# thu-nics/Rad-NeRF

Hardware: AMD Instinct MI355X
Metric: million samples/s fwd+bwd, 8192 rays, model_zoo_size=2; rgb L∞ vs ref (higher is better)
Workload: dtype f16/f32

## Files before the change

### include/radnerf.h

```cpp
#ifndef RADNERF_H
#define RADNERF_H

#include <stdint.h>

#ifdef __cplusplus
extern "C" {
#endif

#define RN_ABI_VERSION 9
#define RN_FX_STATS_BYTES 640
int rn_version(void);
const char* rn_last_error(void);
const char* rn_abi_signatures(void);
void rn_set_debug_flags(int flags);
int rn_debug_cycles(unsigned long long* out);
int rn_set_level_pairing(uint64_t pairing);

int rn_ray_aabb_intersect(const float* rays_o, const float* rays_d, const float* centers,
                          const float* half_sizes, int64_t n_rays, int64_t n_voxels,
                          int32_t max_hits, int32_t* hit_cnt, float* hits_t,
                          int64_t* hits_voxel_idx, void* stream);

int rn_ray_sphere_intersect(const float* rays_o, const float* rays_d, const float* centers,
                            const float* radii, int64_t n_rays, int64_t n_spheres,
// ... 73 lines not shown
                       const float* ts, const int32_t* counts, const int32_t* offsets,
                       int64_t n_rays, int32_t n_models, float T_threshold, int32_t* used,
                       float* opacity_k, float* depth_k, float* rgb_k, float* ws, void* stream);
int rn_ml_combine_fw(const float* gate, const float* opacity_k, const float* depth_k,
                     const float* rgb_k, const float* bg, int64_t n_rays, int32_t n_models,
                     float* rgb, float* opacity, float* depth, void* stream);
int rn_ml_combine_bw(const float* dL_drgb, const float* dL_dopacity, const float* opacity_k,
                     const float* rgb_k, const float* bg, int64_t n_rays, int32_t n_models,
                     float* dL_dgate, void* stream);
int rn_ml_composite_bw(const float* dL_drgb, const float* dL_dopacity, const float* dL_ddepth,
                       const float* gate, const float* bg, const float* sigmas,
                       const float* rgbs, const float* deltas, const float* ts,
                       const int32_t* counts, const int32_t* offsets, const float* opacity_k,
                       const float* depth_k, const float* rgb_k, int64_t n_rays,
                       int32_t n_models, float T_threshold, float* dL_dsigmas, float* dL_drgbs,
                       void* stream);
int rn_ml_composite_dist_fw(const float* sigmas, const float* rgbs, const float* deltas,
                            const float* ts, const int32_t* counts, const int32_t* offsets,
                            int64_t n_rays, int32_t n_models, float T_threshold, int32_t* used,
                            float* opacity_k, float* depth_k, float* rgb_k, float* ws,
                            float* dist_k, void* stream);
int rn_ml_composite_dist_bw(const float* dL_drgb, const float* dL_dopacity,
                            const float* dL_ddepth, const float* dL_ddist, float dL_ddist_const,
                            const float* gate, const float* bg, const float* sigmas,
                            const float* rgbs, const float* deltas, const float* ts,
                            const float* ws, const int32_t* counts, const int32_t* offsets,
                            const float* opacity_k, const float* depth_k, const float* rgb_k,
                            const float* dist_k, int64_t n_rays, int32_t n_models,
                            float T_threshold, float* dL_dsigmas, float* dL_drgbs, void* stream);

int rn_field_fwd(const float* xyzs, const float* dirs, int64_t n_samples, const float* ts,
                 const int32_t* ray_of, const float* rays_o, const float* rays_d,
                 const int32_t* seg_base, const int32_t* seg_count, int32_t n_models,
                 const void* grid_f16, const uint32_t* level_offset, const uint32_t* level_hsize,
                 const uint32_t* level_res, const float* level_scale, const float* xyz_min,
                 const float* extent, const void* frags, float* sigma, float* rgb,
                 void* feat_cache, int32_t blocks_per_model, void* stream);
int rn_field_bwd(const float* xyzs, const float* dirs, int64_t n_samples, const float* ts,
                 const int32_t* ray_of, const float* rays_o, const float* rays_d,
                 const int32_t* seg_base, const int32_t* seg_count, int32_t n_models,
                 const void* grid_f16, const uint32_t* level_offset, const uint32_t* level_hsize,
                 const uint32_t* level_res, const float* level_scale, const float* xyz_min,
                 const float* extent, const void* frags, const float* dL_dsigma,
                 const float* dL_drgb, float* grid_grad, float* dw, const void* feat_cache,
                 int32_t blocks_per_model, void* stream);

int rn_bwd_plan(const int32_t* counts, const int32_t* offsets, const int32_t* seg_base,
                const int32_t* seg_count, const float* ts, int64_t n_rays, int32_t n_models,
                int32_t head_chunks, int32_t head_size, int32_t max_chunk, int32_t min_chunk,
                int32_t balance_blocks, int32_t cap_chunks, int32_t* mstart, int32_t* perm,
                int32_t* chunk_first, int32_t* chunk_desc, int32_t* queue, const float* rays_o,
                const float* rays_d, const float* xyz_min, const float* extent, float* prep,
                void* stream);
int rn_field_bwd_merged(const float* ts, const int32_t* ray_of, const float* rays_o,
                        const float* rays_d, const int32_t* seg_base, const int32_t* seg_count,
                        const int32_t* mstart, const int32_t* perm,
                        const int32_t* chunk_desc, int32_t* queue, int64_t n_rays,
                        int32_t n_models, int32_t max_samples,
                        const void* grid_f16, const uint32_t* level_offset,
                        const uint32_t* level_hsize, const uint32_t* level_res,
                        const float* level_scale, const float* xyz_min, const float* extent,
                        const void* frags, const float* dL_dsigma, const float* dL_drgb,
                        float* grid_grad, float* dw, const void* feat_cache, float* scratch,
                        int64_t scratch_rows, float* park, int32_t max_chunk, int32_t blocks,
                        int32_t* igrad_lo, int32_t* igrad_carry, const float* igrad_scale,
                        int32_t* fx_acc, const float* fx_scale, uint32_t* fx_stats,
                        const int32_t* fx_redo, int32_t fx_mode, void* gb_ctl,
                        uint32_t* gb_page_meta, uint64_t* gb_pages, int32_t gb_pool_pages,
                        void* stream);

int rn_grid_fx_fold(const uint32_t* level_offset, const uint32_t* level_hsize,
                    const uint32_t* level_res, int32_t* fx_acc, const float* fx_scale_cur,
                    float* fx_scale_next, uint32_t* fx_vmax, int32_t* fx_redo, float* grid_grad,
                    void* stream);

int rn_debug_gb_cycles(unsigned long long* out);
int rn_grid_bin_layout(int32_t* out);
int rn_grid_slice_bits(const uint32_t* level_hsize, int32_t* out);
int rn_grid_record_encode(const float* x, int64_t n, uint32_t* out);
int rn_grid_record_decode(const uint32_t* f, int64_t n, int64_t* out);
int rn_grid_bin(const uint32_t* level_hsize, void* ctl, const uint32_t* page_meta,
                const uint64_t* pages_in, uint64_t* pages_out, uint32_t* desc,
                uint32_t* level_pages, int32_t pool_pages, int32_t blocks, void* stream);
int rn_grid_bin_check(const uint32_t* level_hsize, void* ctl, const uint32_t* page_meta,
                      const uint64_t* pages_in, uint64_t* pages_out, uint32_t* desc,
                      uint32_t* level_pages, int32_t pool_pages, const float* fx_scale_cur,
                      float* fx_scale_next, uint32_t* fx_stats, int32_t* fx_redo, void* stream);
int rn_grid_binned_fold(const uint32_t* level_offset, const uint32_t* level_hsize, void* ctl,
                        const uint32_t* page_meta, const uint64_t* pages_in, uint64_t* pages_out,
                        uint32_t* desc, uint32_t* level_pages, int32_t pool_pages,
                        const float* fx_scale_cur, float* fx_scale_next, uint32_t* fx_stats,
                        int32_t* fx_redo, float* grid_grad, void* stream);
int rn_grid_sum(const uint32_t* level_offset, const uint32_t* level_hsize, const void* ctl,
                const uint32_t* desc, const uint32_t* level_pages, const uint64_t* pages_out,
                int32_t pool_pages, const float* fx_scale, const int32_t* redo, float* grid_grad,
                int32_t level_lo, int32_t level_hi, void* stream);

int rn_render_test(const float* rays_o, const float* rays_d, const float* hits_t, int64_t n_rays,
                   int32_t n_models, const uint8_t* density_bitfields, int64_t bitfield_bytes,
                   int32_t cascades, float scale, float exp_step_factor, int32_t grid_size,
                   int32_t max_samples, const void* grid_f16, const uint32_t* level_offset,
                   const uint32_t* level_hsize, const uint32_t* level_res,
                   const float* level_scale, const float* xyz_min, const float* extent,
                   const void* frags, float T_threshold, float* opacity, float* depth,
                   float* rgb, int32_t* n_samples, int32_t blocks, void* stream);

// ... 247 lines not shown
```

### rad-nerf_amd/csrc/field_plan.hip

```cpp
#include "rn_field.h"
#include "rn_merge.h"
#pragma clang fp contract(off)

namespace {

#define PLAN_WAVES 4
#define PLAN_LDS 2048

#define PLAN_UNR 8

struct PlanPrep {
    float4* prep;
    const float* rays_o; const float* rays_d;
    float mn[3], ext[3];
    float inv[3];
};
struct RayPos { float o[3], d[3]; };
__device__ __forceinline__ RayPos plan_ray(const PlanPrep& P, int r) {
    RayPos q;
#pragma unroll
    for (int c = 0; c < 3; ++c) { q.o[c] = P.rays_o[3 * r + c]; q.d[c] = P.rays_d[3 * r + c]; }
    return q;
}
__device__ __forceinline__ void plan_prep_write(const PlanPrep& P, const RayPos& q, int pos,
                                                float t, int s) {
    const float x = fmaf(t, q.d[0], q.o[0]), y = fmaf(t, q.d[1], q.o[1]), z = fmaf(t, q.d[2], q.o[2]);
    auto u = [&](float v, int c) {
        return P.inv[0] != 0.f ? fminf(fmaxf((v - P.mn[c]) * P.inv[c], 0.0f), 1.0f)
                               : unit_coord(v, P.mn[c], P.ext[c]);
    };
    P.prep[pos] = make_float4(u(x, 0), u(y, 1), u(z, 2), __int_as_float(s));
}

__device__ __forceinline__ void plan_ray_runs(int K, int B, int r, const int32_t* __restrict__ counts,
                                              const int32_t* __restrict__ offsets,
                                              const int32_t* __restrict__ seg_base, int* cnt,
                                              int* off, int& ms) {
    int c[MB_KMAX], o[MB_KMAX], sb[MB_KMAX];
#pragma unroll
    for (int k = 0; k < MB_KMAX; ++k) {
        const int kk = k < K ? k : K - 1;
        c[k] = counts[kk * B + r]; o[k] = offsets[kk * B + r]; sb[k] = seg_base[kk];
    }
    ms = 0;
#pragma unroll
    for (int k = 0; k < MB_KMAX; ++k) {
        cnt[k] = k < K ? c[k] : 0;
        off[k] = k < K ? o[k] : 0;
        ms += k < K ? o[k] - sb[k] : 0;
    }
}
__device__ __forceinline__ void plan_stage(int K, int tot_r, const int* bnd, const int* off,
                                           const float* __restrict__ ts, float* st, uint16_t* si) {
    const int lane = rn_lane();
    for (int i0 = 0; i0 < tot_r; i0 += RN_WAVE * PLAN_UNR) {
        float v[PLAN_UNR];
#pragma unroll
        for (int u = 0; u < PLAN_UNR; ++u) {
            const int i = i0 + u * RN_WAVE + lane;
            int base = off[0];
#pragma unroll
            for (int kq = 1; kq < MB_KMAX; ++kq)
                base = (kq < K && i >= bnd[kq]) ? off[kq] - bnd[kq] : base;
            v[u] = i < tot_r ? ts[base + i] : 0.f;
        }
#pragma unroll
        for (int u = 0; u < PLAN_UNR; ++u) {
            const int i = i0 + u * RN_WAVE + lane;
            if (i < tot_r) {
                st[i] = v[u];
                if (si) si[i] = (uint16_t)i;
            }
        }
    }
}

__global__ void __launch_bounds__(PLAN_WAVES * 64)
k_bwd_plan(int B, int K, const int32_t* __restrict__ counts, const int32_t* __restrict__ offsets,
           const int32_t* __restrict__ seg_base, const int32_t* __restrict__ seg_count,
           const float* __restrict__ ts, int32_t* __restrict__ mstart, int32_t* __restrict__ perm,
           PlanPrep P) {
    __shared__ float sT[PLAN_WAVES][PLAN_LDS];
    const int wid = __builtin_amdgcn_readfirstlane(threadIdx.x / RN_WAVE);
    const int r = blockIdx.x * PLAN_WAVES + wid;
    if (r >= B) return;
    const int lane = rn_lane();
    int ms = 0, tot_r = 0;
    int cnt[MB_KMAX], off[MB_KMAX], loc[MB_KMAX];
    plan_ray_runs(K, B, r, counts, offsets, seg_base, cnt, off, ms);
#pragma unroll
    for (int k = 0; k < MB_KMAX; ++k) { loc[k] = tot_r; tot_r += cnt[k]; }
    if (lane == 0) {
        mstart[r] = ms;
        if (r == 0) {
            int tot = 0;
            for (int k = 0; k < K; ++k) tot += seg_count[k];
            mstart[B] = tot;
        }
    }
    const bool staged = tot_r <= PLAN_LDS;
    float* st = sT[wid];
    const RayPos rq = P.prep ? plan_ray(P, r) : RayPos{};
    if (staged) {
        plan_stage(K, tot_r, loc, off, ts, st, nullptr);
        __builtin_amdgcn_wave_barrier();
        __builtin_amdgcn_fence(__ATOMIC_ACQ_REL, "wavefront");
    }
    if (K == 2 && staged) {
        const float* A = st + loc[0];
        const float* Bv = st + loc[1];
        const int nA = cnt[0], nB = cnt[1], n = nA + nB;
        const int L = (n + RN_WAVE - 1) / RN_WAVE;
        const int d = min(lane * L, n);
        int lo = max(0, d - nB), hi = min(d, nA);
        while (lo < hi) {
            const int mid = (lo + hi) >> 1;
            if (A[mid] <= Bv[d - 1 - mid]) lo = mid + 1; else hi = mid;
        }
        int a = lo, b = d - lo;
        const int e = min(d + L, n);
        for (int q = d; q < e; ++q) {
            const bool takeA = a < nA && (b >= nB || A[a] <= Bv[b]);
            const int smp = takeA ? off[0] + a : off[1] + b;
            perm[ms + q] = smp;
            if (P.prep) plan_prep_write(P, rq, ms + q, takeA ? A[a] : Bv[b], smp);
            a += takeA ? 1 : 0;
            b += takeA ? 0 : 1;
        }
        return;
    }
    for (int k = 0; k < K; ++k) {
        for (int i = lane; i < cnt[k]; i += RN_WAVE) {
            const float t = staged ? st[loc[k] + i] : ts[off[k] + i];
            int pos = i;
            for (int k2 = 0; k2 < K; ++k2) {
                if (k2 == k) continue;
                int lo = 0, hi = cnt[k2];
                while (lo < hi) {
                    const int mid = (lo + hi) >> 1;
                    const float t2 = staged ? st[loc[k2] + mid] : ts[off[k2] + mid];
                    if (t2 < t || (k2 < k && t2 == t)) lo = mid + 1; else hi = mid;
                }
                pos += lo;
            }
            perm[ms + pos] = off[k] + i;
            if (P.prep) plan_prep_write(P, rq, ms + pos, t, off[k] + i);
        }
    }
}

#define PLANM_WAVES 2
#define PLANM_LDS 2048

__device__ __forceinline__ void merge_pair_wave(const float* tA, const uint16_t* iA, int nA,
                                                const float* tB, const uint16_t* iB, int nB,
                                                float* to, uint16_t* io, int32_t* gout,
                                                const int* kb, const int* ko, int K,
                                                const PlanPrep& P, const RayPos& rq, int gpos) {
    const int lane = rn_lane();
    const int n = nA + nB;
    const int L = (n + RN_WAVE - 1) / RN_WAVE;
    const int d = min(lane * L, n);
    int lo = max(0, d - nB), hi = min(d, nA);
    while (lo < hi) {
        const int mid = (lo + hi) >> 1;
        if (tA[mid] <= tB[d - 1 - mid]) lo = mid + 1; else hi = mid;
    }
    int a = lo, b = d - lo;
    const int e = min(d + L, n);
    for (int q = d; q < e; ++q) {
        const float ta = tA[a], tb = tB[b];
        const int ja = iA[a], jb = iB[b];
        const bool takeA = a < nA && (b >= nB || ta <= tb);
        const int idx = takeA ? ja : jb;
        if (gout) {
            int base = ko[0];
#pragma unroll
            for (int j = 1; j < MB_KMAX; ++j)
                if (j < K && idx >= kb[j]) base = ko[j] - kb[j];
            gout[q] = base + idx;
            if (P.prep) plan_prep_write(P, rq, gpos + q, takeA ? ta : tb, base + idx);
        } else {
            to[q] = takeA ? ta : tb;
            io[q] = (uint16_t)idx;
        }
        a += takeA ? 1 : 0;
        b += takeA ? 0 : 1;
    }
}

__global__ void __launch_bounds__(PLANM_WAVES * 64)
k_bwd_plan_multi(int B, int K, const int32_t* __restrict__ counts,
                 const int32_t* __restrict__ offsets, const int32_t* __restrict__ seg_base,
                 const int32_t* __restrict__ seg_count, const float* __restrict__ ts,
                 int32_t* __restrict__ mstart, int32_t* __restrict__ perm, PlanPrep P) {
    __shared__ float sT[PLANM_WAVES][2][PLANM_LDS + 2];
    __shared__ uint16_t sI[PLANM_WAVES][2][PLANM_LDS + 2];
    static_assert(PLANM_LDS <= 65536, "u16 sample ids");
    const int wid = __builtin_amdgcn_readfirstlane(threadIdx.x / RN_WAVE);
    const int r = blockIdx.x * PLANM_WAVES + wid;
    if (r >= B) return;
    const int lane = rn_lane();
    int ms = 0, tot_r = 0;
    int bnd[MB_KMAX + 1], off[MB_KMAX], cnt[MB_KMAX];
    plan_ray_runs(K, B, r, counts, offsets, seg_base, cnt, off, ms);
#pragma unroll
    for (int k = 0; k < MB_KMAX; ++k) { bnd[k] = tot_r; tot_r += cnt[k]; }
    bnd[MB_KMAX] = tot_r;
    const RayPos rq = P.prep ? plan_ray(P, r) : RayPos{};
    if (lane == 0) {
        mstart[r] = ms;
        if (r == 0) {
            int tot = 0;
            for (int k = 0; k < K; ++k) tot += seg_count[k];
            mstart[B] = tot;
        }
    }
    if (tot_r > PLANM_LDS) {
        for (int k = 0; k < K; ++k) {
            const int ck = bnd[k + 1] - bnd[k];
            for (int i = lane; i < ck; i += RN_WAVE) {
                const float t = ts[off[k] + i];
                int pos = i;
                for (int k2 = 0; k2 < K; ++k2) {
                    if (k2 == k) continue;
                    int lo = 0, hi = bnd[k2 + 1] - bnd[k2];
                    while (lo < hi) {
                        const int mid = (lo + hi) >> 1;
                        const float t2 = ts[off[k2] + mid];
                        if (t2 < t || (k2 < k && t2 == t)) lo = mid + 1; else hi = mid;
                    }
                    pos += lo;
                }
                perm[ms + pos] = off[k] + i;
                if (P.prep) plan_prep_write(P, rq, ms + pos, t, off[k] + i);
            }
        }
        return;
    }
    int cur = 0;
    int kb[MB_KMAX];
#pragma unroll
    for (int k = 0; k < MB_KMAX; ++k) kb[k] = k < K ? bnd[k] : 0;
    plan_stage(K, tot_r, bnd, off, ts, sT[wid][0], sI[wid][0]);
    int nr = K;
    while (true) {
        __builtin_amdgcn_wave_barrier();
        __builtin_amdgcn_fence(__ATOMIC_ACQ_REL, "wavefront");
        const bool last = nr <= 2;
        const float* ts_ = sT[wid][cur];
        const uint16_t* is_ = sI[wid][cur];
        for (int p = 0; 2 * p < nr; ++p) {
            const int a0 = bnd[2 * p], a1 = bnd[min(2 * p + 1, nr)], b1 = bnd[min(2 * p + 2, nr)];
            merge_pair_wave(ts_ + a0, is_ + a0, a1 - a0, ts_ + a1, is_ + a1, b1 - a1,
                            sT[wid][cur ^ 1] + a0, sI[wid][cur ^ 1] + a0,
                            nullptr, kb, off, K, P, rq, ms + a0);
        }
        if (last) {
            __builtin_amdgcn_wave_barrier();
            __builtin_amdgcn_fence(__ATOMIC_ACQ_REL, "wavefront");
            const float* to = sT[wid][cur ^ 1];
            const uint16_t* io = sI[wid][cur ^ 1];
            for (int q = lane; q < tot_r; q += RN_WAVE) {
                const int idx = io[q];
                int base = off[0];
#pragma unroll
                for (int jk = 1; jk < MB_KMAX; ++jk)
                    if (jk < K && idx >= kb[jk]) base = off[jk] - kb[jk];
                perm[ms + q] = base + idx;
                if (P.prep) plan_prep_write(P, rq, ms + q, to[q], base + idx);
            }
            return;
        }
        const int nn = (nr + 1) / 2;
        for (int p = 0; p < nn; ++p) bnd[p] = bnd[2 * p];
        bnd[nn] = bnd[nr];
        nr = nn;
        cur ^= 1;
    }
}

struct ChunkPlan {
    int head_n, head, max_chunk, min_chunk, c1, n;
    __host__ __device__ int hbound(int c) const {
        return head_n > 0 ? (int)(((int64_t)head * c * (c + 1)) / (2 * (int64_t)head_n)) : 0;
    }
    __host__ __device__ int bound(int c) const {
        const int H = hbound(head_n);
        if (c < head_n) return hbound(c);
        if (c <= c1) return H + (c - head_n) * max_chunk;
        return H + (c1 - head_n) * max_chunk + (c - c1) * min_chunk;
    }
};

__host__ __device__ __forceinline__ ChunkPlan chunk_plan(int total, int head_n, int head,
                                                         int max_chunk, int min_chunk, int blocks) {
    ChunkPlan p;
// ... 8 lines not shown
    if (blocks > 0 && main_end > H) {
        const int64_t main = main_end - H, per = (int64_t)blocks * max_chunk;
        const int64_t m = (main + per - 1) / per;
        const int64_t sz = (main + (int64_t)blocks * m - 1) / ((int64_t)blocks * m);
        p.max_chunk = (int)(sz < min_chunk ? min_chunk : (sz > max_chunk ? max_chunk : sz));
    }
    p.c1 = p.head_n + (main_end > H ? (main_end - H) / p.max_chunk : 0);
    const int rest = total - p.bound(p.c1);
    p.n = p.c1 + (rest > 0 ? (rest + min_chunk - 1) / min_chunk : 0);
    return p;
}

__global__ void __launch_bounds__(256)
k_bwd_chunks(int B, int K, const int32_t* __restrict__ mstart,
             const int32_t* __restrict__ offsets, const int32_t* __restrict__ seg_base,
             const int32_t* __restrict__ seg_count, int head_n, int head, int max_chunk,
             int min_chunk, int blocks, int cap_chunks, int32_t* __restrict__ chunk_first,
             int32_t* __restrict__ desc, int32_t* __restrict__ queue) {
    const int c = blockIdx.x * blockDim.x + threadIdx.x;
    const int total = mstart[B];
    const ChunkPlan p = chunk_plan(total, head_n, head, max_chunk, min_chunk, blocks);
    const int n = min(p.n, cap_chunks);
    if (c == 0) { queue[0] = 0; queue[1] = n; queue[2] = 0; }
    if (c > n) return;
    auto first_ray = [&](int cc) {
        if (cc == p.n) return B;
        const int bound = p.bound(cc);
        int lo = 0, hi = B;
        while (lo < hi) {
            const int mid = (lo + hi) >> 1;
            if (mstart[mid] < bound) lo = mid + 1; else hi = mid;
        }
        return lo;
    };
    if (c == n) { chunk_first[c] = first_ray(c); return; }
    const int first[2] = {first_ray(c), first_ray(c + 1)};
    chunk_first[c] = first[0];
    int32_t* d = desc + (size_t)c * CH_DESC;
    const int r0 = first[0], r1 = first[1];
    d[CH_R0] = r0; d[CH_R1] = r1; d[2] = 0; d[3] = 0;
    for (int k = 0; k < MB_KMAX; ++k) {
        int a0 = 0, cnt = 0;
        if (k < K && r0 < B) {
            a0 = offsets[k * B + r0];
            const int a1 = r1 < B ? offsets[k * B + r1] : seg_base[k] + seg_count[k];
            cnt = a1 - a0;
        }
        d[ch_first(k)] = a0; d[ch_count(k)] = cnt;
    }
}

}

extern "C" {

int rn_bwd_plan(const int32_t* counts, const int32_t* offsets, const int32_t* seg_base,
                const int32_t* seg_count, const float* ts, int64_t n_rays, int32_t n_models,
                int32_t head_chunks, int32_t head_size, int32_t max_chunk, int32_t min_chunk,
                int32_t balance_blocks, int32_t cap_chunks, int32_t* mstart, int32_t* perm,
                int32_t* chunk_first, int32_t* chunk_desc, int32_t* queue, const float* rays_o,
                const float* rays_d, const float* xyz_min, const float* extent, float* prep,
                void* stream) {
    RN_CHECK_ARG(n_rays >= 1 && n_models >= 1 && n_models <= MB_KMAX, "bad sizes");
    RN_CHECK_ARG(max_chunk >= min_chunk && min_chunk >= 1 && cap_chunks >= 1 && head_chunks >= 0 &&
                 head_size >= 0 && head_size <= max_chunk && balance_blocks >= 0,
                 "bad chunk sizes");
    RN_CHECK_ARG(counts && offsets && seg_base && seg_count && ts && mstart && perm &&
                 chunk_first && chunk_desc && queue, "null pointer");
    RN_CHECK_ARG(!prep || (rays_o && rays_d && xyz_min && extent), "null pointer (prep)");
    PlanPrep P{};
    P.prep = (float4*)prep; P.rays_o = rays_o; P.rays_d = rays_d;
    if (prep) {
        bool pow2 = true;
        for (int c = 0; c < 3; ++c) {
            P.mn[c] = xyz_min[c]; P.ext[c] = extent[c];
            int e;
            pow2 = pow2 && extent[c] > 0.f && std::frexp(extent[c], &e) == 0.5f &&
                   e > -120 && e < 120;
        }
        for (int c = 0; c < 3; ++c) P.inv[c] = pow2 ? 1.0f / extent[c] : 0.f;
    }
    if (n_models > 2)
        k_bwd_plan_multi<<<nblk(n_rays, PLANM_WAVES), PLANM_WAVES * 64, 0, (hipStream_t)stream>>>(
            (int)n_rays, n_models, counts, offsets, seg_base, seg_count, ts, mstart, perm, P);
    else
        k_bwd_plan<<<nblk(n_rays, PLAN_WAVES), PLAN_WAVES * 64, 0, (hipStream_t)stream>>>(
            (int)n_rays, n_models, counts, offsets, seg_base, seg_count, ts, mstart, perm, P);
    RN_CHECK_LAUNCH();
    k_bwd_chunks<<<nblk(cap_chunks + 1, 256), 256, 0, (hipStream_t)stream>>>(
        (int)n_rays, n_models, mstart, offsets, seg_base, seg_count, head_chunks, head_size,
        max_chunk, min_chunk, balance_blocks, cap_chunks, chunk_first, chunk_desc, queue);
    RN_CHECK_LAUNCH();
    return 0;
}

}
```

### rad-nerf_amd/radnerf_amd/_lib.py

```python
import ctypes
import os

_HERE = os.path.dirname(os.path.abspath(__file__))
LIB_PATH = os.environ.get("RADNERF_LIB", os.path.join(_HERE, "librn.so"))
ABLATION_LIB_PATH = os.environ.get("RADNERF_ABL_LIB", os.path.join(_HERE, "librn_abl.so"))

P = ctypes.c_void_p
I32 = ctypes.c_int32
I64 = ctypes.c_int64
F32 = ctypes.c_float
F64 = ctypes.c_double
U64 = ctypes.c_uint64

SIGNATURES = {
    "rn_ray_aabb_intersect": [P, P, P, P, I64, I64, I32, P, P, P, P],
    "rn_ray_sphere_intersect": [P, P, P, P, I64, I64, I32, P, P, P, P],
    "rn_raymarching_train_bw": [P, P, P, P, I64, P, P, P],
    "rn_ml_march_bw": [P, P, I64, I32, P, P, P, P, P, P],
    "rn_field_dinput": [P, P, I64, P, P, P, P, P, P, I32, P, P, P, P, P, P, P, P, P, P, P, P, P,
                        P, I32, P],
    "rn_field_density": [P, I64, P, P, P, P, P, P, P, P, P, P, P],
    "rn_debug_cycles": [P],
    "rn_set_level_pairing": [ctypes.c_uint64],
    "rn_density_update_sampled": [P, P, I32, I32, I32, F32, F32, F32, U64, P, P, P, P, P, P, P,
                                  P, P, P, P, P, P, I32, P],
    "rn_density_update_visible": [P, P, I32, I32, I32, F32, F32, F32, U64, P, P, P, P, P, P, P,
                                  P, P, P, P, P, P, I32, P, I32, P],
    "rn_distortion_loss_fw": [P, P, P, P, I64, P, P, P, P],
    "rn_distortion_loss_bw": [P, P, P, P, P, P, P, I64, P, P],
    "rn_raymarching_train_count": [P, P, P, P, I32, F32, F32, P, I32, I32, I64, P, P],
    "rn_raymarching_train_write": [P, P, P, P, I32, F32, F32, P, I32, I32, I64, P, P, P, P, P,
                                   P, P, P],
    "rn_scan_segments": [P, I32, I64, I32, P, P, P, P, P],
    "rn_raymarching_test": [P, P, P, P, I64, P, I32, F32, F32, I32, I32, I32, P, P, P, P, P, P],
    "rn_ml_march_count": [P, P, P, P, F32, P, P, I64, I32, I32, F32, F32, I32, I32, I64, P, P, P,
                          P],
    "rn_ml_compact": [P, P, I64, I32, I32, P, P, P, P, P, P],
    "rn_ml_march_write": [P, P, P, P, F32, P, P, I64, I32, I32, F32, F32, I32, I32, I64, P, P,
                          P, P, P, P],
    "rn_composite_train_fw": [P, P, P, P, P, I64, F32, P, P, P, P, P, P],
    "rn_composite_train_bw": [P, P, P, P, P, P, P, P, P, P, I64, P, P, P, F32, P, P, P],
    "rn_composite_test_fw": [P, P, P, P, I64, I32, P, F32, P, P, P, P, P],
    "rn_ml_composite_fw": [P, P, P, P, P, P, I64, I32, F32, P, P, P, P, P, P],
    "rn_ml_combine_fw": [P, P, P, P, P, I64, I32, P, P, P, P],
    "rn_ml_combine_bw": [P, P, P, P, P, I64, I32, P, P],
    "rn_ml_composite_bw": [P, P, P, P, P, P, P, P, P, P, P, P, P, P, I64, I32, F32, P, P, P],
    "rn_ml_composite_dist_fw": [P, P, P, P, P, P, I64, I32, F32, P, P, P, P, P, P, P],
    "rn_ml_composite_dist_bw": [P, P, P, P, F32, P, P, P, P, P, P, P, P, P, P, P, P, P, I64, I32,
                                F32, P, P, P],
    "rn_field_fwd": [P, P, I64, P, P, P, P, P, P, I32, P, P, P, P, P, P, P, P, P, P, P, I32, P],
    "rn_field_bwd": [P, P, I64, P, P, P, P, P, P, I32, P, P, P, P, P, P, P, P, P, P, P, P, P,
                     I32, P],
    "rn_bwd_plan": [P, P, P, P, P, I64, I32, I32, I32, I32, I32, I32, I32, P, P, P, P, P,
                    P, P, P, P, P, P],
    "rn_field_bwd_merged": [P, P, P, P, P, P, P, P, P, P, I64, I32, I32, P, P, P, P, P, P,
                            P, P, P, P, P, P, P, P, I64, P, I32, I32, P, P, P, P, P, P,
                            P, I32, P, P, P, I32, P],
    "rn_grid_fx_fold": [P, P, P, P, P, P, P, P, P, P],
    "rn_grid_bin_layout": [P],
    "rn_debug_gb_cycles": [P],
    "rn_grid_slice_bits": [P, P],
    "rn_grid_record_encode": [P, I64, P],
    "rn_grid_record_decode": [P, I64, P],
    "rn_grid_bin": [P, P, P, P, P, P, P, I32, I32, P],
    "rn_grid_sum": [P, P, P, P, P, P, I32, P, P, P, I32, I32, P],
    "rn_grid_bin_check": [P, P, P, P, P, P, P, I32, P, P, P, P, P],
    "rn_grid_binned_fold": [P, P, P, P, P, P, P, P, I32, P, P, P, P, P, P],
    "rn_render_test": [P, P, P, I64, I32, P, I64, I32, F32, F32, I32, I32, P, P, P, P, P, P, P,
                       P, F32, P, P, P, P, I32, P],
    "rn_gate_select": [P, I64, I32, F32, I32, I32, P, P, P, P, P, P, P, P, P, P],
    "rn_render_test_list": [P, P, P, I64, I32, P, I64, I32, F32, F32, I32, I32, P, P, P, P, P, P,
                            P, P, F32, P, P, P, P, P, P, I32, P],
    "rn_ml_march_count_list": [P, P, P, P, F32, P, P, I64, I32, I32, F32, F32, I32, I32, I64, P,
                               P, P, P, P, P],
    "rn_gate_select_bw": [P, P, P, I64, I32, I32, P, P],
    "rn_nerf_loss_routed": [P, P, P, P, P, P, P, I64, I32, F32, F32, F32, P, P, P, P, P, P],
    "rn_nerf_loss_routed_det": [P, P, P, P, P, P, P, I64, I32, F32, F32, F32, P, P, P, P, P, P,
                                P],
    "rn_seed_scale": [P, P, I32, P, P, P, P, P, P],
    "rn_igrad_to_f32": [I64, P, P, P, P, P],
    "rn_field_fwd_merged": [P, P, P, P, P, P, P, P, I64, I32, P, P, P, P, P, P, P, P, P, P, P,
                            P, P, I32, I32, P],
    "rn_field_fwd_levels": [P, P, P, P, P, P, I64, I32, P, P, P, P, P, P, P, P, P, P, P, P, P,
                            P, I64, P, I32, I32, I32, P, P],
    "rn_gate_fwd": [P, P, I32, I64, I32, P, P, P, I32, P],
    "rn_gate_bwd": [P, P, I32, I64, I32, P, P, P, I32, P, P, I32, P],
    "rn_nerf_loss": [P, P, P, P, P, P, I64, I32, F32, F32, F32, P, P, P, P, P, P],
    "rn_adam": [P, P, P, P, I64, F64, F64, F64, F64, I32, F32, P, I64, P],
    "rn_reduce_partials": [P, I32, I64, P, P],
    "rn_colsum_ordered": [P, I64, I32, P, P],
    "rn_field_bwd_merged_det": [P, P, P, P, P, P, P, P, P, P, I64, I32, I32, P, P, P, P, P, P,
                                P, P, P, P, P, P, P, P, I64, P, I32, I32, P, P, P, P],
    "rn_gate_bwd_det": [P, P, I32, I64, I32, P, P, P, I32, P, P, I32, P],
    "rn_nerf_loss_det": [P, P, P, P, P, P, I64, I32, F32, F32, F32, P, P, P, P, P, P, P],
    "rn_get_rays": [P, P, P, P, I64, P, P, P, P, P],
    "rn_get_rays_pose": [P, P, P, P, P, P, I64, P, P, P, P, P],
    "rn_get_rays_pose_bw": [P, P, P, P, P, I64, I64, P, P, P, P, P, P, P],
    "rn_sample_batch": [P, I32, I64, I64, P, P, P, P, P, U64, I64, I32, I64, I32, P, P, P, P, P,
                        P, P, P, P],
    "rn_guided_weights": [P, I64, I32, I32, I32, P, P, P, P],
    "rn_sample_batch_guided": [P, I32, I64, I64, P, P, P, P, P, U64, I64, I32, I64, I32, P, P, P,
                               P, P, P, P, P, I32, I32, I32, F32, P, P, P, P, P],
    "rn_guided_epilogue": [P, P, P, P, I64, I32, I64, P, P, P, P, P, P],
    "rn_guided_refresh": [P, P, P, I64, F32, P],
    "rn_ml_combine_test": [P, P, P, P, P, I64, I32, I64, P, P, P, P, P],
    "rn_image_sse": [P, P, I64, P, P, P],
    "rn_ssim": [P, P, I32, I32, I32, P, P, P, P],
# ... 130 lines not shown
```

### rad-nerf_amd/radnerf_amd/fused.py

```python
import collections

import torch

from . import layout as LY
from . import sparse_gate
from ._lib import GATE_SELECT_WORK_BYTES, lib
from .networks import field_ptrs, model_bitfields

MAX_SAMPLES = 1024
NEAR_DISTANCE = 0.01
SEG_ALIGN = 128
FX_STATS_BYTES = 640
GM_F32, GM_FX, GM_FX_REDO, GM_BIN, GM_BIN_F32 = 0, 2, 3, 4, 5
NO_IG, NO_FX, NO_GB = (None, None, None), (None, None, None, None, GM_F32), (None, None, None, 0)


GB_SUM_FAULT = 18
GB_CTL_READ = GB_SUM_FAULT + 1


def clamp_split(split_level):
    return max(0, min(15, int(split_level)))


# ... 284 lines not shown
        return route_params("FusedMLRenderer", self.gate.out_dim, gate_topk, gate_min,
                            renormalize, self._route_always)

    def forward(self, rays_o, rays_d, gate_in2, noise, bg, T_threshold=1e-4,
                exp_step_factor=0.0, distortion=False, gate_topk=None, gate_min=0.0,
                renormalize=False):
        m, g, w, L = self.model, self.gate, self.ws, lib()
        B, K, G = rays_o.shape[0], m.size, g.out_dim
        assert B == w.B and noise.shape == (K, B)
        routed = self._routed = self.route_params(gate_topk, gate_min, renormalize)
        st = _stream(rays_o.device)
        out_gate = torch.empty(B, G, device=rays_o.device)
        imp = torch.zeros(G, device=rays_o.device)
        side = self._side(rays_o.device)
        main = torch.cuda.current_stream(rays_o.device)
        if G == 1:
            out_gate.fill_(1.0)
            imp.fill_(float(B))
            side.wait_stream(main)
        else:
            frags = g.packed_frags()
            side.wait_stream(main)
            self._ev("gate_fwd", L.gate_fwd, rays_o.data_ptr(), gate_in2.data_ptr(), 3, B, G,
                     frags.data_ptr(), out_gate.data_ptr(),
                     None if self.deterministic else imp.data_ptr(),
                     max(1, min(256, (B + 127) // 128)), side.cuda_stream, stream=side)
            if self.deterministic:
                self._ev("gate_colsum", L.colsum_ordered, out_gate.data_ptr(), B, G,
                         imp.data_ptr(), side.cuda_stream, stream=side)
        rt = None
        if routed is not None:
            rt = w.route_buffers()
            self._ev("gate_select", L.gate_select, out_gate.data_ptr(), B, G, routed[1],
                     routed[0], int(routed[2]), rt["live"].data_ptr(),
                     rt["gate_used"].data_ptr(), rt["list"].data_ptr(), rt["count"].data_ptr(),
                     None, None, None, None, rt["work"].data_ptr(), side.cuda_stream,
                     stream=side)
            main.wait_stream(side)
        bits = self.bitfields()
        march = (rays_o.data_ptr(), rays_d.data_ptr(), m.center.data_ptr(),
                 m.half_size.data_ptr(), NEAR_DISTANCE, noise.data_ptr(), bits.data_ptr(),
                 self.bitfield_bytes, K, m.cascades, float(m.scale), float(exp_step_factor),
                 m.grid_size, MAX_SAMPLES, B)
        if rt is None:
            self._ev("march", L.ml_march_count, *march, w.counts.data_ptr(),
                     w.stage_ts.data_ptr(), w.stage_dt.data_ptr(), st)
        else:
            self._ev("march", L.ml_march_count_list, *march, w.counts.data_ptr(),
                     w.stage_ts.data_ptr(), w.stage_dt.data_ptr(), rt["list"].data_ptr(),
                     rt["count"].data_ptr(), st)
        self._ev("scan", L.scan_segments, w.counts.data_ptr(), K, B, SEG_ALIGN,
                 w.offsets.data_ptr(), w.seg_base.data_ptr(), w.seg_count.data_ptr(),
                 w.meta.data_ptr(), st)
        self._ev("compact", L.ml_compact, w.counts.data_ptr(), w.offsets.data_ptr(), B, K,
                 MAX_SAMPLES, w.stage_ts.data_ptr(), w.stage_dt.data_ptr(), w.ts.data_ptr(),
                 w.deltas.data_ptr(), w.ray_of.data_ptr(), st)
        if self.merged_bwd or self.merged_fwd:
            self._plan(st, rays_o, rays_d if self.level_fwd and self.plan_prep else None)
        self._field_fwd(rays_o, rays_d, st)
        comp = (w.sigma.data_ptr(), w.rgb.data_ptr(), w.deltas.data_ptr(),
                w.ts.data_ptr(), w.counts.data_ptr(), w.offsets.data_ptr(), B, K,
                float(T_threshold), w.used.data_ptr(), w.opacity_k.data_ptr(),
                w.depth_k.data_ptr(), w.rgb_k.data_ptr(), w.ws.data_ptr())
        self._dist_forward = bool(distortion)
        if distortion:
            self._ev("composite_dist_fw", L.ml_composite_dist_fw, *comp, w.dist_k.data_ptr(), st)
        else:
            self._ev("composite_fw", L.ml_composite_fw, *comp, st)
        ok, dk, rk = self._gather_model_outputs()
        rgb = torch.empty(B, 3, device=rays_o.device)
        opacity = torch.empty(B, device=rays_o.device)
        depth = torch.empty(B, G, device=rays_o.device)
        main.wait_stream(side)
        out_gate.record_stream(side)
        imp.record_stream(side)
        weights = out_gate if rt is None else rt["gate_used"]
        self._ev("combine_fw", L.ml_combine_fw, weights.data_ptr(), ok.data_ptr(), dk.data_ptr(),
                        rk.data_ptr(), bg.data_ptr(), B, G, rgb.data_ptr(),
                        opacity.data_ptr(), depth.data_ptr(), st)
        return rgb, opacity, depth, out_gate, imp

    def _gather_model_outputs(self):
        return self._model_outputs()

    def _model_outputs(self):
        w = self.ws
        return w.opacity_k, w.depth_k, w.rgb_k

    def _local_cols(self, x):
        return x

    def _plan_params(self):
        return (self.max_chunk, min(self.min_chunk, self.max_chunk),
                self.merged_blocks if self.head_chunk else 0,
                min(self.head_chunk, self.max_chunk),
                self.merged_blocks if self.balance_chunks else 0)

    def _plan(self, st, rays_o=None, rays_d=None):
        w, L, m = self.ws, lib(), self.model
        prep = w.level_buffers(st)[1] if rays_d is not None else None
        key = max_chunk, min_chunk, head_n, head, bal = self._plan_params()
        self._cap_chunks, self._chunks = w.chunk_list(max_chunk, min_chunk, head_n, bal)
        self._ev("bwd_plan", L.bwd_plan, w.counts.data_ptr(), w.offsets.data_ptr(),
                 w.seg_base.data_ptr(), w.seg_count.data_ptr(), w.ts.data_ptr(), w.B, w.K,
                 head_n, head, max_chunk, min_chunk, bal, self._cap_chunks,
                 w.mstart.data_ptr(), w.perm.data_ptr(), self._chunks.data_ptr(),
                 w._chunk_desc.data_ptr(), w.queue.data_ptr(),
                 *((None,) * 5 if prep is None else
                   (rays_o.data_ptr(), rays_d.data_ptr(), m._h_min.ctypes.data,
                    m._h_ext.ctypes.data, prep.data_ptr())), st)
        self._plan_key = key
        self._prep_ready = prep is not None

    def _sample_ptrs(self, rays_o, rays_d):
        w = self.ws
        return (w.ts.data_ptr(), w.ray_of.data_ptr(), rays_o.data_ptr(), rays_d.data_ptr(),
                w.seg_base.data_ptr(), w.seg_count.data_ptr())

    def _field(self, fwd, rays_o, rays_d, st, grid_grad=None, dw=None):
        return (self._field_fwd(rays_o, rays_d, st) if fwd else
                self._field_bwd(rays_o, rays_d, st, grid_grad, dw))

    def _field_fwd(self, rays_o, rays_d, st):
        m, w, L = self.model, self.ws, lib()
        samples, grid = self._sample_ptrs(rays_o, rays_d), field_ptrs(m)
        out = (w.sigma.data_ptr(), w.rgb.data_ptr())
        feat = w.feat.data_ptr() if self.feat_cache else None
        if self.level_fwd and (self.merged_bwd or self.merged_fwd):
            planes, prep = w.level_buffers(st)
            self._ev("field_fwd", L.field_fwd_levels, *samples, w.B, m.size, *grid, *out,
                     w.feat.data_ptr(), w.mstart.data_ptr(), w.perm.data_ptr(),
                     planes.data_ptr(), planes.shape[1], prep.data_ptr(), int(self._prep_ready),
                     self.level_enc_blocks, self.level_mlp_blocks, None, st)
            self._prep_ready = False
        elif self.merged_fwd:
            order = ((w.mstart.data_ptr(), w.perm.data_ptr())
                     if self.feat_cache and self.merged_encode else (None, None))
            self._ev("field_fwd", L.field_fwd_merged, *samples, w._chunk_desc.data_ptr(),
                     w.queue.data_ptr(), w.B, m.size, *grid, *out, feat, *order,
                     self.merged_fwd_blocks, self.merged_fwd_threads, st)
        else:
            self._ev("field_fwd", L.field_fwd, None, None, 0, *samples, m.size, *grid, *out, feat,
                     self.fwd_blocks, st)

    def _field_bwd(self, rays_o, rays_d, st, grid_grad, dw):
        m, w, L = self.model, self.ws, lib()
        samples, grid = self._sample_ptrs(rays_o, rays_d), field_ptrs(m)
        feat = w.feat.data_ptr() if self.feat_cache else None
        if not self.merged_bwd:
            return self._bwd_f32(lambda name: self._ev(
                name, L.field_bwd, None, None, 0, *samples, m.size, *grid, w.dsigma.data_ptr(),
                w.drgb.data_ptr(), grid_grad.data_ptr(), dw.data_ptr(), feat, self.bwd_blocks, st))
        rows, scratch, park = w.bwd_scratch(self.merged_blocks, self.max_chunk)
        if self._plan_key != self._plan_params():
            self._plan(st)
        head = (*samples, w.mstart.data_ptr(), w.perm.data_ptr(), w._chunk_desc.data_ptr(),
                w.queue.data_ptr(), w.B, m.size, MAX_SAMPLES, *grid, w.dsigma.data_ptr(),
                w.drgb.data_ptr(), grid_grad.data_ptr())
        tail = (feat, scratch.data_ptr(), rows, park.data_ptr(), self.max_chunk, self.merged_blocks)

        def launch(name, ig=NO_IG, fx=NO_FX, gb=NO_GB, dw_part=None):
            if dw_part is not None:
                self._ev(name, L.field_bwd_merged_det, *head, dw_part.data_ptr(), *tail, *ig, st)
# ... 444 lines not shown
```

Measured before the change: 1216.

## Fuse sample compaction into the backward plan kernel reading staged buffers

The separate compact kernel, which copied staged per-model ts/deltas into packed arrays and filled ray_of, is folded into the plan kernel. The plan now reads the staged buffers directly and writes the compacted outputs while loading ts into LDS. That saves one launch and one global round trip of ts. The K=2 merge path is also restructured: it records merge order in LDS first, then writes perm and prep coalesced across lanes. This adds stores and LDS use to the plan kernel, which can reduce its occupancy.

After: 1221 (median of 6 runs). No clear change (+0.4%).

```diff
diff --git a/include/radnerf.h b/include/radnerf.h
--- a/include/radnerf.h
+++ b/include/radnerf.h
@@ -149,6 +149,15 @@
                 int32_t* chunk_first, int32_t* chunk_desc, int32_t* queue, const float* rays_o,
                 const float* rays_d, const float* xyz_min, const float* extent, float* prep,
                 void* stream);
+int rn_bwd_plan_staged(const int32_t* counts, const int32_t* offsets, const int32_t* seg_base,
+                       const int32_t* seg_count, float* ts, int64_t n_rays, int32_t n_models,
+                       int32_t head_chunks, int32_t head_size, int32_t max_chunk,
+                       int32_t min_chunk, int32_t balance_blocks, int32_t cap_chunks,
+                       int32_t* mstart, int32_t* perm, int32_t* chunk_first, int32_t* chunk_desc,
+                       int32_t* queue, const float* rays_o, const float* rays_d,
+                       const float* xyz_min, const float* extent, float* prep,
+                       int32_t max_samples, const float* stage_ts, const float* stage_deltas,
+                       float* deltas, int32_t* ray_of, void* stream);
 int rn_field_bwd_merged(const float* ts, const int32_t* ray_of, const float* rays_o,
                         const float* rays_d, const int32_t* seg_base, const int32_t* seg_count,
                         const int32_t* mstart, const int32_t* perm,
diff --git a/rad-nerf_amd/csrc/field_plan.hip b/rad-nerf_amd/csrc/field_plan.hip
--- a/rad-nerf_amd/csrc/field_plan.hip
+++ b/rad-nerf_amd/csrc/field_plan.hip
@@ -50,37 +50,77 @@
         ms += k < K ? o[k] - sb[k] : 0;
     }
 }
+struct PlanStage {
+    const float* sts; const float* sdt;
+    float* ts; float* deltas; int32_t* ray_of;
+    int max_samples;
+};
+__device__ __forceinline__ int64_t stage_run(const PlanStage& S, int B, int k, int r) {
+    return ((int64_t)k * B + r) * S.max_samples;
+}
+
+template <bool STG, int KM, int UNR>
 __device__ __forceinline__ void plan_stage(int K, int tot_r, const int* bnd, const int* off,
-                                           const float* __restrict__ ts, float* st, uint16_t* si) {
+                                           const float* __restrict__ ts, float* st, uint16_t* si,
+                                           const PlanStage& S, int B, int r) {
     const int lane = rn_lane();
-    for (int i0 = 0; i0 < tot_r; i0 += RN_WAVE * PLAN_UNR) {
-        float v[PLAN_UNR];
-#pragma unroll
-        for (int u = 0; u < PLAN_UNR; ++u) {
-            const int i = i0 + u * RN_WAVE + lane;
+    for (int i0 = 0; i0 < tot_r; i0 += RN_WAVE * UNR) {
+        float v[UNR], dv[UNR];
+        int dst[UNR];
+#pragma unroll
+        for (int u = 0; u < UNR; ++u) {
+            const int i = i0 + u * RN_WAVE + lane, ic = STG ? min(i, tot_r - 1) : i;
             int base = off[0];
-#pragma unroll
-            for (int kq = 1; kq < MB_KMAX; ++kq)
-                base = (kq < K && i >= bnd[kq]) ? off[kq] - bnd[kq] : base;
-            v[u] = i < tot_r ? ts[base + i] : 0.f;
-        }
-#pragma unroll
-        for (int u = 0; u < PLAN_UNR; ++u) {
+            int kr = 0, b0 = 0;
+#pragma unroll
+            for (int kq = 1; kq < KM; ++kq) {
+                const bool in = kq < K && ic >= bnd[kq];
+                base = in ? off[kq] - bnd[kq] : base;
+                kr = in ? kq : kr;
+                b0 = in ? bnd[kq] : b0;
+            }
+            if (STG) {
+                const int64_t src = stage_run(S, B, kr, r) + (ic - b0);
+                v[u] = S.sts[src];
+                dv[u] = S.sdt[src];
+                dst[u] = base + i;
+            } else {
+                v[u] = i < tot_r ? ts[base + i] : 0.f;
+            }
+        }
+#pragma unroll
+        for (int u = 0; u < UNR; ++u) {
             const int i = i0 + u * RN_WAVE + lane;
             if (i < tot_r) {
                 st[i] = v[u];
                 if (si) si[i] = (uint16_t)i;
+                if (STG) { S.ts[dst[u]] = v[u]; S.deltas[dst[u]] = dv[u]; S.ray_of[dst[u]] = r; }
             }
         }
     }
 }
 
+__device__ __forceinline__ void plan_copy_runs(int K, int B, int r, const int* cnt, const int* off,
+                                               const PlanStage& S) {
+    for (int k = 0; k < K; ++k) {
+        const int64_t src = stage_run(S, B, k, r);
+        for (int i = rn_lane(); i < cnt[k]; i += RN_WAVE) {
+            S.ts[off[k] + i] = S.sts[src + i];
+            S.deltas[off[k] + i] = S.sdt[src + i];
+            S.ray_of[off[k] + i] = r;
+        }
+    }
+}
+
+template <bool STG>
 __global__ void __launch_bounds__(PLAN_WAVES * 64)
 k_bwd_plan(int B, int K, const int32_t* __restrict__ counts, const int32_t* __restrict__ offsets,
            const int32_t* __restrict__ seg_base, const int32_t* __restrict__ seg_count,
            const float* __restrict__ ts, int32_t* __restrict__ mstart, int32_t* __restrict__ perm,
-           PlanPrep P) {
+           PlanPrep P, PlanStage S) {
     __shared__ float sT[PLAN_WAVES][PLAN_LDS];
+    __shared__ uint16_t sOrd[PLAN_WAVES][PLAN_LDS];
+    static_assert(PLAN_LDS <= 65536, "u16 positions");
     const int wid = __builtin_amdgcn_readfirstlane(threadIdx.x / RN_WAVE);
     const int r = blockIdx.x * PLAN_WAVES + wid;
     if (r >= B) return;
@@ -102,14 +142,20 @@
     float* st = sT[wid];
     const RayPos rq = P.prep ? plan_ray(P, r) : RayPos{};
     if (staged) {
-        plan_stage(K, tot_r, loc, off, ts, st, nullptr);
+        plan_stage<STG, STG ? 2 : MB_KMAX, PLAN_UNR>(K, tot_r, loc, off, ts, st, nullptr, S, B, r);
         __builtin_amdgcn_wave_barrier();
         __builtin_amdgcn_fence(__ATOMIC_ACQ_REL, "wavefront");
-    }
+    } else if (STG) {
+        plan_copy_runs(K, B, r, cnt, off, S);
+    }
+    auto gts = [&](int k2, int i) {
+        return STG ? S.sts[stage_run(S, B, k2, r) + i] : ts[off[k2] + i];
+    };
     if (K == 2 && staged) {
         const float* A = st + loc[0];
         const float* Bv = st + loc[1];
         const int nA = cnt[0], nB = cnt[1], n = nA + nB;
+        uint16_t* ord = sOrd[wid];
         const int L = (n + RN_WAVE - 1) / RN_WAVE;
         const int d = min(lane * L, n);
         int lo = max(0, d - nB), hi = min(d, nA);
@@ -121,24 +167,30 @@
         const int e = min(d + L, n);
         for (int q = d; q < e; ++q) {
             const bool takeA = a < nA && (b >= nB || A[a] <= Bv[b]);
-            const int smp = takeA ? off[0] + a : off[1] + b;
-            perm[ms + q] = smp;
-            if (P.prep) plan_prep_write(P, rq, ms + q, takeA ? A[a] : Bv[b], smp);
+            ord[q] = (uint16_t)(takeA ? a : nA + b);
             a += takeA ? 1 : 0;
             b += takeA ? 0 : 1;
         }
+        __builtin_amdgcn_wave_barrier();
+        __builtin_amdgcn_fence(__ATOMIC_ACQ_REL, "wavefront");
+        for (int q = lane; q < n; q += RN_WAVE) {
+            const int idx = ord[q];
+            const int smp = idx < nA ? off[0] + idx : off[1] + idx - nA;
+            perm[ms + q] = smp;
+            if (P.prep) plan_prep_write(P, rq, ms + q, st[idx], smp);
+        }
         return;
     }
     for (int k = 0; k < K; ++k) {
         for (int i = lane; i < cnt[k]; i += RN_WAVE) {
-            const float t = staged ? st[loc[k] + i] : ts[off[k] + i];
+            const float t = staged ? st[loc[k] + i] : gts(k, i);
             int pos = i;
             for (int k2 = 0; k2 < K; ++k2) {
                 if (k2 == k) continue;
                 int lo = 0, hi = cnt[k2];
                 while (lo < hi) {
                     const int mid = (lo + hi) >> 1;
-                    const float t2 = staged ? st[loc[k2] + mid] : ts[off[k2] + mid];
+                    const float t2 = staged ? st[loc[k2] + mid] : gts(k2, mid);
                     if (t2 < t || (k2 < k && t2 == t)) lo = mid + 1; else hi = mid;
                 }
                 pos += lo;
@@ -189,11 +241,13 @@
     }
 }
 
+template <bool STG>
 __global__ void __launch_bounds__(PLANM_WAVES * 64)
 k_bwd_plan_multi(int B, int K, const int32_t* __restrict__ counts,
                  const int32_t* __restrict__ offsets, const int32_t* __restrict__ seg_base,
                  const int32_t* __restrict__ seg_count, const float* __restrict__ ts,
-                 int32_t* __restrict__ mstart, int32_t* __restrict__ perm, PlanPrep P) {
+                 int32_t* __restrict__ mstart, int32_t* __restrict__ perm, PlanPrep P,
+                 PlanStage S) {
     __shared__ float sT[PLANM_WAVES][2][PLANM_LDS + 2];
     __shared__ uint16_t sI[PLANM_WAVES][2][PLANM_LDS + 2];
     static_assert(PLANM_LDS <= 65536, "u16 sample ids");
@@ -217,17 +271,21 @@
         }
     }
     if (tot_r > PLANM_LDS) {
+        if (STG) plan_copy_runs(K, B, r, cnt, off, S);
+        auto gts = [&](int k2, int i) {
+            return STG ? S.sts[stage_run(S, B, k2, r) + i] : ts[off[k2] + i];
+        };
         for (int k = 0; k < K; ++k) {
             const int ck = bnd[k + 1] - bnd[k];
             for (int i = lane; i < ck; i += RN_WAVE) {
-                const float t = ts[off[k] + i];
+                const float t = gts(k, i);
                 int pos = i;
                 for (int k2 = 0; k2 < K; ++k2) {
                     if (k2 == k) continue;
                     int lo = 0, hi = bnd[k2 + 1] - bnd[k2];
                     while (lo < hi) {
                         const int mid = (lo + hi) >> 1;
-                        const float t2 = ts[off[k2] + mid];
+                        const float t2 = gts(k2, mid);
                         if (t2 < t || (k2 < k && t2 == t)) lo = mid + 1; else hi = mid;
                     }
                     pos += lo;
@@ -242,7 +300,8 @@
     int kb[MB_KMAX];
 #pragma unroll
     for (int k = 0; k < MB_KMAX; ++k) kb[k] = k < K ? bnd[k] : 0;
-    plan_stage(K, tot_r, bnd, off, ts, sT[wid][0], sI[wid][0]);
+    plan_stage<STG, MB_KMAX, STG ? PLAN_UNR / 2 : PLAN_UNR>(K, tot_r, bnd, off, ts, sT[wid][0],
+                                                            sI[wid][0], S, B, r);
     int nr = K;
     while (true) {
         __builtin_amdgcn_wave_barrier();
@@ -357,6 +416,48 @@
 
 }
 
+static int bwd_plan_launch(const char* who, const int32_t* counts, const int32_t* offsets,
+                           const int32_t* seg_base, const int32_t* seg_count, const float* ts,
+                           const PlanStage& S,
+                           int64_t n_rays, int32_t n_models, int32_t head_chunks,
+                           int32_t head_size, int32_t max_chunk, int32_t min_chunk,
+                           int32_t balance_blocks, int32_t cap_chunks, int32_t* mstart,
+                           int32_t* perm, int32_t* chunk_first, int32_t* chunk_desc,
+                           int32_t* queue, const float* rays_o, const float* rays_d,
+                           const float* xyz_min, const float* extent, float* prep, void* stream) {
+    PlanPrep P{};
+    P.prep = (float4*)prep; P.rays_o = rays_o; P.rays_d = rays_d;
+    if (prep) {
+        bool pow2 = true;
+        for (int c = 0; c < 3; ++c) {
+            P.mn[c] = xyz_min[c]; P.ext[c] = extent[c];
+            int e;
+            pow2 = pow2 && extent[c] > 0.f && std::frexp(extent[c], &e) == 0.5f &&
+                   e > -120 && e < 120;
+        }
+        for (int c = 0; c < 3; ++c) P.inv[c] = pow2 ? 1.0f / extent[c] : 0.f;
+    }
+    hipStream_t st = (hipStream_t)stream;
+    const int B = (int)n_rays;
+#define RN_PLAN_ARGS B, n_models, counts, offsets, seg_base, seg_count, ts, mstart, perm, P, S
+    if (n_models > 2) {
+        const dim3 g(nblk(n_rays, PLANM_WAVES)), b(PLANM_WAVES * 64);
+        if (S.sts) k_bwd_plan_multi<true><<<g, b, 0, st>>>(RN_PLAN_ARGS);
+        else k_bwd_plan_multi<false><<<g, b, 0, st>>>(RN_PLAN_ARGS);
+    } else {
+        const dim3 g(nblk(n_rays, PLAN_WAVES)), b(PLAN_WAVES * 64);
+        if (S.sts) k_bwd_plan<true><<<g, b, 0, st>>>(RN_PLAN_ARGS);
+        else k_bwd_plan<false><<<g, b, 0, st>>>(RN_PLAN_ARGS);
+    }
+#undef RN_PLAN_ARGS
+    RN_CHECK_LAUNCH_AS(who);
+    k_bwd_chunks<<<nblk(cap_chunks + 1, 256), 256, 0, st>>>(
+        (int)n_rays, n_models, mstart, offsets, seg_base, seg_count, head_chunks, head_size,
+        max_chunk, min_chunk, balance_blocks, cap_chunks, chunk_first, chunk_desc, queue);
+    RN_CHECK_LAUNCH_AS(who);
+    return 0;
+}
+
 extern "C" {
 
 int rn_bwd_plan(const int32_t* counts, const int32_t* offsets, const int32_t* seg_base,
@@ -373,30 +474,37 @@
     RN_CHECK_ARG(counts && offsets && seg_base && seg_count && ts && mstart && perm &&
                  chunk_first && chunk_desc && queue, "null pointer");
     RN_CHECK_ARG(!prep || (rays_o && rays_d && xyz_min && extent), "null pointer (prep)");
-    PlanPrep P{};
-    P.prep = (float4*)prep; P.rays_o = rays_o; P.rays_d = rays_d;
-    if (prep) {
-        bool pow2 = true;
-        for (int c = 0; c < 3; ++c) {
-            P.mn[c] = xyz_min[c]; P.ext[c] = extent[c];
-            int e;
-            pow2 = pow2 && extent[c] > 0.f && std::frexp(extent[c], &e) == 0.5f &&
-                   e > -120 && e < 120;
-        }
-        for (int c = 0; c < 3; ++c) P.inv[c] = pow2 ? 1.0f / extent[c] : 0.f;
-    }
-    if (n_models > 2)
-        k_bwd_plan_multi<<<nblk(n_rays, PLANM_WAVES), PLANM_WAVES * 64, 0, (hipStream_t)stream>>>(
-            (int)n_rays, n_models, counts, offsets, seg_base, seg_count, ts, mstart, perm, P);
-    else
-        k_bwd_plan<<<nblk(n_rays, PLAN_WAVES), PLAN_WAVES * 64, 0, (hipStream_t)stream>>>(
-            (int)n_rays, n_models, counts, offsets, seg_base, seg_count, ts, mstart, perm, P);
-    RN_CHECK_LAUNCH();
-    k_bwd_chunks<<<nblk(cap_chunks + 1, 256), 256, 0, (hipStream_t)stream>>>(
-        (int)n_rays, n_models, mstart, offsets, seg_base, seg_count, head_chunks, head_size,
-        max_chunk, min_chunk, balance_blocks, cap_chunks, chunk_first, chunk_desc, queue);
-    RN_CHECK_LAUNCH();
-    return 0;
-}
-
-}
+    return bwd_plan_launch(__func__, counts, offsets, seg_base, seg_count, ts, PlanStage{}, n_rays,
+                           n_models, head_chunks, head_size, max_chunk, min_chunk, balance_blocks,
+                           cap_chunks, mstart, perm, chunk_first, chunk_desc, queue, rays_o,
+                           rays_d, xyz_min, extent, prep, stream);
+}
+
+int rn_bwd_plan_staged(const int32_t* counts, const int32_t* offsets, const int32_t* seg_base,
+                       const int32_t* seg_count, float* ts, int64_t n_rays, int32_t n_models,
+                       int32_t head_chunks, int32_t head_size, int32_t max_chunk,
+                       int32_t min_chunk, int32_t balance_blocks, int32_t cap_chunks,
+                       int32_t* mstart, int32_t* perm, int32_t* chunk_first, int32_t* chunk_desc,
+                       int32_t* queue, const float* rays_o, const float* rays_d,
+                       const float* xyz_min, const float* extent, float* prep,
+                       int32_t max_samples, const float* stage_ts, const float* stage_deltas,
+                       float* deltas, int32_t* ray_of, void* stream) {
+    RN_CHECK_ARG(n_rays >= 1 && n_models >= 1 && n_models <= MB_KMAX && max_samples >= 1,
+                 "bad sizes");
+    RN_CHECK_ARG(max_chunk >= min_chunk && min_chunk >= 1 && cap_chunks >= 1 && head_chunks >= 0 &&
+                 head_size >= 0 && head_size <= max_chunk && balance_blocks >= 0,
+                 "bad chunk sizes");
+    RN_CHECK_ARG(counts && offsets && seg_base && seg_count && stage_ts && stage_deltas && ts &&
+                 deltas && ray_of && mstart && perm && chunk_first && chunk_desc && queue,
+                 "null pointer");
+    RN_CHECK_ARG(!prep || (rays_o && rays_d && xyz_min && extent), "null pointer (prep)");
+    PlanStage S{};
+    S.sts = stage_ts; S.sdt = stage_deltas; S.ts = ts; S.deltas = deltas; S.ray_of = ray_of;
+    S.max_samples = max_samples;
+    return bwd_plan_launch(__func__, counts, offsets, seg_base, seg_count, nullptr, S, n_rays,
+                           n_models, head_chunks, head_size, max_chunk, min_chunk, balance_blocks,
+                           cap_chunks, mstart, perm, chunk_first, chunk_desc, queue, rays_o,
+                           rays_d, xyz_min, extent, prep, stream);
+}
+
+}
diff --git a/rad-nerf_amd/radnerf_amd/_lib.py b/rad-nerf_amd/radnerf_amd/_lib.py
--- a/rad-nerf_amd/radnerf_amd/_lib.py
+++ b/rad-nerf_amd/radnerf_amd/_lib.py
@@ -53,6 +53,8 @@
                      I32, P],
     "rn_bwd_plan": [P, P, P, P, P, I64, I32, I32, I32, I32, I32, I32, I32, P, P, P, P, P,
                     P, P, P, P, P, P],
+    "rn_bwd_plan_staged": [P, P, P, P, P, I64, I32, I32, I32, I32, I32, I32, I32, P, P, P, P, P,
+                           P, P, P, P, P, I32, P, P, P, P, P],
     "rn_field_bwd_merged": [P, P, P, P, P, P, P, P, P, P, I64, I32, I32, P, P, P, P, P, P,
                             P, P, P, P, P, P, P, P, I64, P, I32, I32, P, P, P, P, P, P,
                             P, I32, P, P, P, I32, P],
diff --git a/rad-nerf_amd/radnerf_amd/fused.py b/rad-nerf_amd/radnerf_amd/fused.py
--- a/rad-nerf_amd/radnerf_amd/fused.py
+++ b/rad-nerf_amd/radnerf_amd/fused.py
@@ -360,11 +360,13 @@
         self._ev("scan", L.scan_segments, w.counts.data_ptr(), K, B, SEG_ALIGN,
                  w.offsets.data_ptr(), w.seg_base.data_ptr(), w.seg_count.data_ptr(),
                  w.meta.data_ptr(), st)
-        self._ev("compact", L.ml_compact, w.counts.data_ptr(), w.offsets.data_ptr(), B, K,
-                 MAX_SAMPLES, w.stage_ts.data_ptr(), w.stage_dt.data_ptr(), w.ts.data_ptr(),
-                 w.deltas.data_ptr(), w.ray_of.data_ptr(), st)
         if self.merged_bwd or self.merged_fwd:
-            self._plan(st, rays_o, rays_d if self.level_fwd and self.plan_prep else None)
+            self._plan(st, rays_o, rays_d if self.level_fwd and self.plan_prep else None,
+                       staged=True)
+        else:
+            self._ev("compact", L.ml_compact, w.counts.data_ptr(), w.offsets.data_ptr(), B, K,
+                     MAX_SAMPLES, w.stage_ts.data_ptr(), w.stage_dt.data_ptr(), w.ts.data_ptr(),
+                     w.deltas.data_ptr(), w.ray_of.data_ptr(), st)
         self._field_fwd(rays_o, rays_d, st)
         comp = (w.sigma.data_ptr(), w.rgb.data_ptr(), w.deltas.data_ptr(),
                 w.ts.data_ptr(), w.counts.data_ptr(), w.offsets.data_ptr(), B, K,
@@ -404,19 +406,22 @@
                 min(self.head_chunk, self.max_chunk),
                 self.merged_blocks if self.balance_chunks else 0)
 
-    def _plan(self, st, rays_o=None, rays_d=None):
+    def _plan(self, st, rays_o=None, rays_d=None, staged=False):
         w, L, m = self.ws, lib(), self.model
         prep = w.level_buffers(st)[1] if rays_d is not None else None
         key = max_chunk, min_chunk, head_n, head, bal = self._plan_params()
         self._cap_chunks, self._chunks = w.chunk_list(max_chunk, min_chunk, head_n, bal)
-        self._ev("bwd_plan", L.bwd_plan, w.counts.data_ptr(), w.offsets.data_ptr(),
+        self._ev("bwd_plan", L.bwd_plan_staged if staged else L.bwd_plan,
+                 w.counts.data_ptr(), w.offsets.data_ptr(),
                  w.seg_base.data_ptr(), w.seg_count.data_ptr(), w.ts.data_ptr(), w.B, w.K,
                  head_n, head, max_chunk, min_chunk, bal, self._cap_chunks,
                  w.mstart.data_ptr(), w.perm.data_ptr(), self._chunks.data_ptr(),
                  w._chunk_desc.data_ptr(), w.queue.data_ptr(),
                  *((None,) * 5 if prep is None else
                    (rays_o.data_ptr(), rays_d.data_ptr(), m._h_min.ctypes.data,
-                    m._h_ext.ctypes.data, prep.data_ptr())), st)
+                    m._h_ext.ctypes.data, prep.data_ptr())),
+                 *((MAX_SAMPLES, w.stage_ts.data_ptr(), w.stage_dt.data_ptr(),
+                    w.deltas.data_ptr(), w.ray_of.data_ptr()) if staged else ()), st)
         self._plan_key = key
         self._prep_ready = prep is not None
 
```
